# davxy/ark-ec-vrfs

Measured on AMD Instinct MI355X. Metric: Bandersnatch IETF-ECVRF verifies/sec, 2^20 batch per GPU, higher is better.
Workload: dtype u32; 1 GPU; IETF ECVRF verify, Bandersnatch_SHA-512_ELL2, batch 2^20 per GPU, compressed points (161 B/verify), checked decode: on curve + prime-order subgroup, as arkworks' deserialisation, ad="", about 1 in 16 proofs forged (BASELINE.json configs[2]); global_batch=1048576, parallelism=items sharded x1, result gather only, subgroup_check=True

## Files before the change

### ark_ec_vrfs_amd/csrc/fr.cuh

```cuda
#pragma once
#include "fe.cuh"

VRF_NS_BEGIN

template <class C>
VRF_HD void fr_montmul(uint32_t out[8], const uint32_t a[8], const uint32_t b[8]) {
  uint32_t t[10];
#pragma unroll
  for (int i = 0; i < 10; ++i) t[i] = 0;
#pragma unroll
  for (int i = 0; i < 8; ++i) {
    uint64_t c = 0;
#pragma unroll
    for (int j = 0; j < 8; ++j) {
      uint64_t x = (uint64_t)a[j] * b[i] + t[j] + c;
      t[j] = (uint32_t)x;
      c = x >> 32;
    }
    uint64_t x = (uint64_t)t[8] + c;
    t[8] = (uint32_t)x;
    t[9] = (uint32_t)(x >> 32);
    uint32_t m = t[0] * C::R_NINV32;
    c = ((uint64_t)m * C::r32(0) + t[0]) >> 32;
#pragma unroll
// ... 47 lines not shown
  const bool keep = borrow && c == 0;
#pragma unroll
  for (int i = 0; i < 8; ++i) out[i] = keep ? s[i] : d[i];
}

template <class C>
VRF_HD void fr_reduce512(uint32_t out[8], const uint32_t x[16]) {
  uint32_t r1[8], r2[8], lo[8], hi[8];
#pragma unroll
  for (int i = 0; i < 8; ++i) { r1[i] = C::r_r1(i); r2[i] = C::r_r2(i); }
  fr_montmul<C>(lo, x, r1);
  fr_montmul<C>(hi, x + 8, r2);
  fr_add<C>(out, lo, hi);
}

template <class C>
VRF_HD void fr_mul(uint32_t out[8], const uint32_t a[8], const uint32_t b[8]) {
  uint32_t t[8], r2[8];
#pragma unroll
  for (int i = 0; i < 8; ++i) r2[i] = C::r_r2(i);
  fr_montmul<C>(t, a, b);
  fr_montmul<C>(out, t, r2);
}

template <class C>
VRF_HD bool fr_is_canonical(const uint32_t a[8]) {
  bool lt = false, decided = false;
#pragma unroll
  for (int i = 7; i >= 0; --i) {
    uint32_t ri = C::r32(i);
    if (!decided && a[i] != ri) { lt = a[i] < ri; decided = true; }
  }
  return lt;
}

VRF_HD void scalar_recode_signed4(uint32_t out[8], const uint32_t k[8]) {
  uint32_t c = 0;
#pragma unroll
  for (int i = 0; i < 8; ++i) {
    uint64_t x = (uint64_t)k[i] + 0x88888888u + c;
    out[i] = (uint32_t)x;
    c = (uint32_t)(x >> 32);
  }
}
VRF_HD int scalar_digit4(const uint32_t rec[8], int w) {
  uint32_t word = rec[0];
#pragma unroll
  for (int i = 1; i < 8; ++i)
    if ((w >> 3) == i) word = rec[i];
  return (int)((word >> ((w & 7) * 4)) & 15u) - 8;
}

struct GlvHalf {
  uint32_t mag[4];
  bool neg;
};

VRF_HD void acc5_muladd(uint32_t acc[5], const uint32_t x[5], const uint32_t (&y)[5], bool subtract) {
  uint32_t p[5];
  uint64_t carry = 0;
#pragma unroll
  for (int k = 0; k < 5; ++k) {
    uint64_t lo = carry & 0xffffffffu, hi = carry >> 32;
#pragma unroll
    for (int i = 0; i <= k; ++i) {
      uint64_t t = (uint64_t)x[i] * y[k - i];
      lo += t & 0xffffffffu;
      hi += t >> 32;
    }
    p[k] = (uint32_t)lo;
    carry = hi + (lo >> 32);
  }
  uint64_t c = subtract ? 1 : 0;
#pragma unroll
  for (int k = 0; k < 5; ++k) {
    uint64_t t = (uint64_t)acc[k] + (subtract ? ~p[k] : p[k]) + c;
    acc[k] = (uint32_t)t;
    c = t >> 32;
  }
}

VRF_HD void glv_round_mul(uint32_t out[5], const uint32_t k[8], const uint32_t (&g)[5]) {
  uint32_t prod[13];
  uint64_t carry = 0;
#pragma unroll
  for (int col = 0; col < 13; ++col) {
    uint64_t lo = carry & 0xffffffffu, hi = carry >> 32;
#pragma unroll
    for (int i = 0; i < 8; ++i) {
      int j = col - i;
      if (j >= 0 && j < 5) {
        uint64_t t = (uint64_t)k[i] * g[j];
        lo += t & 0xffffffffu;
        hi += t >> 32;
      }
    }
    if (col == 7) lo += 0x80000000u;
    prod[col] = (uint32_t)lo;
    carry = hi + (lo >> 32);
  }
#pragma unroll
  for (int i = 0; i < 5; ++i) out[i] = prod[8 + i];
}

VRF_HD GlvHalf glv_finish(const uint32_t v[5]) {
  GlvHalf h;
  h.neg = (v[4] >> 31) != 0;
  uint64_t c = h.neg ? 1 : 0;
#pragma unroll
  for (int i = 0; i < 4; ++i) {
    uint64_t t = (uint64_t)(h.neg ? ~v[i] : v[i]) + c;
    h.mag[i] = (uint32_t)t;
    c = t >> 32;
  }
  return h;
}

#if VRF_FIELD != 0
VRF_HD void glv_decompose_bs(GlvHalf& k1, GlvHalf& k2, const uint32_t k[8]);
#else
VRF_HD void glv_decompose_bs(GlvHalf& k1, GlvHalf& k2, const uint32_t k[8]) {
  uint32_t c1[5], c2[5];
  glv_round_mul(c1, k, vrfk::BS_GLV_G1);
  glv_round_mul(c2, k, vrfk::BS_GLV_G2);
  uint32_t v1[5], v2[5];
#pragma unroll
  for (int i = 0; i < 5; ++i) { v1[i] = k[i]; v2[i] = 0; }
  acc5_muladd(v1, c1, vrfk::BS_GLV_A1_MAG, !(vrfk::BS_GLV_C1_NEG ^ vrfk::BS_GLV_A1_NEG));
  acc5_muladd(v1, c2, vrfk::BS_GLV_A2_MAG, !(vrfk::BS_GLV_C2_NEG ^ vrfk::BS_GLV_A2_NEG));
  acc5_muladd(v2, c1, vrfk::BS_GLV_B1_MAG, !(vrfk::BS_GLV_C1_NEG ^ vrfk::BS_GLV_B1_NEG));
  acc5_muladd(v2, c2, vrfk::BS_GLV_B2_MAG, !(vrfk::BS_GLV_C2_NEG ^ vrfk::BS_GLV_B2_NEG));
  k1 = glv_finish(v1);
  k2 = glv_finish(v2);
}
#endif

VRF_HD void scalar_recode_signed4_128(uint32_t out[4], const uint32_t k[4]) {
  uint32_t c = 0;
#pragma unroll
  for (int i = 0; i < 4; ++i) {
    uint64_t x = (uint64_t)k[i] + 0x88888888u + c;
    out[i] = (uint32_t)x;
    c = (uint32_t)(x >> 32);
  }
}
VRF_HD int scalar_digit4_128(const uint32_t rec[4], int w) {
  uint32_t word = rec[0];
#pragma unroll
  for (int i = 1; i < 4; ++i)
    if ((w >> 3) == i) word = rec[i];
  return (int)((word >> ((w & 7) * 4)) & 15u) - 8;
}

VRF_NS_END
```

### ark_ec_vrfs_amd/csrc/k_verify.hip

```cpp
#include "kernels.h"
#include "tai_find.cuh"

VRF_NS_BEGIN

template <class S>
VRF_HD void load_cs_reduced(uint32_t c[8], uint32_t s[8]) {
  uint32_t cr[8];
  fr_reduce256<S>(cr, c);
  const bool s_ok = fr_is_canonical<S>(s);
#pragma unroll
  for (int j = 0; j < 8; ++j) { c[j] = s_ok ? cr[j] : 0u; s[j] = s_ok ? s[j] : 0u; }
}

template <class S, int MINW>
__global__ void __launch_bounds__(BLOCK, MINW) k_verify_decode(VerifyArgs a) {
  size_t first = ((size_t)blockIdx.x * BLOCK + threadIdx.x) * a.k_lane;
  if (first >= a.n) return;
  verify_decode_multi<S>(a.k_lane, a.T, first, a.n, a.pk, a.h, a.gamma, a.ws.tabs, a.ws.pts, a.ws.flags, a.check_mask);
}

template <class S>
__global__ void __launch_bounds__(BLOCK, 2) k_verify_input_from_alpha(size_t n, BytesView msg, uint8_t* enc, uint32_t* tabs,
                                                                      DevTables T, const uint8_t* tai_ctr) {
  size_t i = (size_t)blockIdx.x * BLOCK + threadIdx.x;
  if (i >= n) return;
  const uint8_t* m; uint32_t len;
  bytes_get(msg, i, m, len);
  PtE h = data_to_point<S>(m, len, T.sq, tai_ctr ? tai_ctr[i] : 0u);
  FeN x, y;
  te_to_affine(x, y, h);
  uint32_t e[8];
  te_encode_affine(e, x, y, T.sq.str.flags);
  store32(enc, i, e);
  build_glv_tables<S>(tabs + i * (VERIFY_TABS * WIN_TABLE_WORDS) + 2 * WIN_TABLE_WORDS, x, y);
}
template <class S, int MINW>
__global__ void __launch_bounds__(BLOCK, MINW) k_verify_decode_skip_h(VerifyArgs a) {
  size_t first = ((size_t)blockIdx.x * BLOCK + threadIdx.x) * a.k_lane;
  if (first >= a.n) return;
  verify_decode_multi<S, 2, true>(a.k_lane, a.T, first, a.n, a.pk, nullptr, a.gamma, a.ws.tabs, a.ws.pts, a.ws.flags,
                                  a.check_mask);
}

template <class S, int MINW>
__global__ void __launch_bounds__(BLOCK, MINW) k_verify_decode_keyed(VerifyArgs a) {
  size_t first = ((size_t)blockIdx.x * BLOCK + threadIdx.x) * a.k_lane;
  if (first >= a.n) return;
  verify_decode_multi<S, 2>(a.k_lane, a.T, first, a.n, nullptr, a.h, a.gamma, a.ws.tabs, a.ws.pts, a.ws.flags,
                            a.check_mask);
#pragma unroll 1
  for (int k = 0; k < a.k_lane; ++k) {
    const size_t i = first + k;
    if (i >= a.n) break;
    const uint32_t key = a.key_index[i];
    const bool key_ok = key < a.n_keys && a.key_valid[key] != 0;
    if (!key_ok) a.ws.flags[i] = 0;
  }
}

template <class S>
__global__ void __launch_bounds__(BLOCK) k_verify_comb_u(VerifyArgs a) {
  size_t i = (size_t)blockIdx.x * BLOCK + threadIdx.x;
  if (i >= a.n) return;
  uint32_t c[8], s[8];
  load32(c, a.c, i); load32(s, a.s, i);
  load_cs_reduced<S>(c, s);
  const uint32_t key = a.key_index[i] < a.n_keys ? a.key_index[i] : 0;
  PtE r = gcomb_mul<S>(a.T.g_comb, s);
  r = comb_add<S>(r, a.key_combs + (size_t)key * COMB_WORDS, c, true);
  uint32_t* out = a.ws.pts + i * PROVE_PTS_WORDS;
  fe_store(out, r.X); fe_store(out + NL, r.Y); fe_store(out + 2 * NL, r.Z);
}

template <class S>
__global__ void __launch_bounds__(BLOCK) k_verify_decode_affine(VerifyArgs a) {
  size_t i = (size_t)blockIdx.x * BLOCK + threadIdx.x;
  if (i >= a.n) return;
  uint32_t xy[3][16], enc[3][8];
  const uint32_t* p0 = reinterpret_cast<const uint32_t*>(a.pk + i * 64);
  const uint32_t* p1 = reinterpret_cast<const uint32_t*>(a.h + i * 64);
  const uint32_t* p2 = reinterpret_cast<const uint32_t*>(a.gamma + i * 64);
#pragma unroll
  for (int j = 0; j < 16; ++j) { xy[0][j] = p0[j]; xy[1][j] = p1[j]; xy[2][j] = p2[j]; }
  bool ok = verify_decode_affine_item<S>(enc, xy, a.ws.tabs + i * (VERIFY_TABS * WIN_TABLE_WORDS), a.T.sq, a.check_mask,
                                         a.affine_in == 2);
  uint32_t* aux = a.ws.aux + i * AUX_WORDS;
#pragma unroll
  for (int j = 0; j < 8; ++j) { aux[j] = enc[0][j]; aux[8 + j] = enc[1][j]; aux[16 + j] = enc[2][j]; }
  a.ws.flags[i] = ok ? 1 : 0;
}

template <class S, int HALF>
__global__ void __launch_bounds__(BLOCK) k_verify_straus(VerifyArgs a) {
  size_t i = (size_t)blockIdx.x * BLOCK + threadIdx.x;
  if (i >= a.n) return;
  uint32_t c[8], s[8];
  load32(c, a.c, i); load32(s, a.s, i);
  load_cs_reduced<S>(c, s);
  verify_straus_item<S, HALF>(a.ws.pts + i * PROVE_PTS_WORDS + HALF * UV_WORDS, a.T,
                                    a.ws.tabs + i * (VERIFY_TABS * WIN_TABLE_WORDS), c, s);
}

template <class S>
__global__ void __launch_bounds__(BLOCK) k_verify_straus_both(VerifyArgs a) {
  size_t i = (size_t)blockIdx.x * BLOCK + threadIdx.x;
  if (i >= a.n) return;
  uint32_t c[8], s[8];
  load32(c, a.c, i); load32(s, a.s, i);
  load_cs_reduced<S>(c, s);
  const uint32_t* tabs = a.ws.tabs + i * (VERIFY_TABS * WIN_TABLE_WORDS);
  if (blockIdx.y == 0) verify_straus_item<S, 1>(a.ws.pts + i * PROVE_PTS_WORDS + UV_WORDS, a.T, tabs, c, s);
  else verify_straus_item<S, 0>(a.ws.pts + i * PROVE_PTS_WORDS, a.T, tabs, c, s);
}

template <class S, int MINW>
__global__ void __launch_bounds__(BLOCK, MINW) k_verify_finish(VerifyArgs a) {
  size_t first = ((size_t)blockIdx.x * BLOCK + threadIdx.x) * a.k_lane;
  if (first >= a.n) return;
  verify_finish_multi<S>(a.k_lane, first, a.n, a.ws.pts, PROVE_PTS_WORDS, a.pk, a.h, a.gamma,
                         a.affine_in ? a.ws.aux : nullptr, AUX_WORDS, a.c, a.s, a.ad, a.ws.flags, a.status,
                         a.T.sq.str, a.key_index, a.n_keys);
}

template <class S>
static void launch_verify_t(const VerifyArgs& a, hipStream_t st, hipEvent_t* ev) {
  const size_t lanes_k_ = (a.n + a.k_lane - 1) / a.k_lane;
  const dim3 gk = grid_for(lanes_k_);
  if (ev) (void)hipEventRecord(ev[0], st);
  if (a.key_index) VRF_LAUNCH_MINW(k_verify_decode_keyed, S, lanes_k_, gk, spread_lds_bytes(gk.x), st, a);
  else if (a.h_in_tabs) VRF_LAUNCH_MINW(k_verify_decode_skip_h, S, lanes_k_, gk, spread_lds_bytes(gk.x), st, a);
  else if (a.affine_in) hipLaunchKernelGGL(k_verify_decode_affine<S>, grid_for(a.n), dim3(BLOCK), 0, st, a);
  else VRF_LAUNCH_MINW(k_verify_decode, S, lanes_k_, gk, spread_lds_bytes(gk.x), st, a);
  if (!ev && !a.key_index && a.n <= STRAUS_FUSE_MAX_ITEMS) {
    dim3 g2 = grid_for(a.n);
    g2.y = 2;
    hipLaunchKernelGGL(k_verify_straus_both<S>, g2, dim3(BLOCK), 0, st, a);
    if (a.u_out) { launch_test_verify_uv_readout(a, st); return; }
    VRF_LAUNCH_MINW(k_verify_finish, S, lanes_k_, gk, spread_lds_bytes(gk.x), st, a);
    return;
  }
  if (ev) (void)hipEventRecord(ev[1], st);
  hipLaunchKernelGGL((k_verify_straus<S, 1>), grid_for(a.n), dim3(BLOCK), 0, st, a);
  if (ev) (void)hipEventRecord(ev[2], st);
  if (a.key_index) hipLaunchKernelGGL(k_verify_comb_u<S>, grid_for(a.n), dim3(BLOCK), 0, st, a);
  else hipLaunchKernelGGL((k_verify_straus<S, 0>), grid_for(a.n), dim3(BLOCK), 0, st, a);
  if (ev) (void)hipEventRecord(ev[3], st);
  if (a.u_out) { launch_test_verify_uv_readout(a, st); return; }
  VRF_LAUNCH_MINW(k_verify_finish, S, lanes_k_, gk, spread_lds_bytes(gk.x), st, a);
  if (ev) (void)hipEventRecord(ev[4], st);
}
void launch_verify_input_from_alpha(int suite, size_t n, BytesView msg, uint8_t* enc, uint32_t* tabs, DevTables T,
                                    hipStream_t st, uint8_t* tai_ctr, unsigned long long* queue) {
  if (!n) return;
  VRF_DISPATCH_SUITE(suite, {
    const uint8_t* ctr = nullptr;
    if constexpr (!S::H2C_ELL2) {
      if (tai_ctr && queue) { launch_tai_find_t<S>(n, msg, tai_ctr, T.sq, queue, st); ctr = tai_ctr; }
    }
    hipLaunchKernelGGL(k_verify_input_from_alpha<S>, grid_for(n), dim3(BLOCK), 0, st, n, msg, enc, tabs, T, ctr);
  });
}
void launch_ietf_verify(const VerifyArgs& a, hipStream_t st, hipEvent_t* ev) {
  if (a.n == 0) return;
  VRF_DISPATCH_SUITE(a.suite, launch_verify_t<S>(a, st, ev));
}

VRF_NS_END
```

### ark_ec_vrfs_amd/csrc/vrf_core.cuh

```cuda
#pragma once
#include "fe.cuh"
#include "fr.cuh"
#include "sha512.cuh"
#include "te.cuh"

VRF_NS_BEGIN

enum : uint32_t { ST_OK = 0, ST_VERIFICATION_FAILURE = 1, ST_INVALID_DATA = 2 };


constexpr int WIN_ENTRIES = 8;
constexpr int WIN_TABLE_WORDS = WIN_ENTRIES * PTC_WORDS;

enum : int { SUBGROUP_2DESCENT = 0, SUBGROUP_TATE8 = 1, SUBGROUP_ORDER = 2, SUBGROUP_HALVE_TATE4 = 3 };

#if VRF_FIELD == 0
struct SuiteBS : CurveBS {
  static constexpr bool HAS_GLV = true;
  static constexpr int SUBGROUP = SUBGROUP_2DESCENT;
  static constexpr bool H2C_ELL2 = true;
};

struct SuiteJJ : CurveJJ {
  static constexpr bool HAS_GLV = false;
// ... 456 lines not shown
  }
  start = te_add_cached<C>(start, step, false);
  comb_chain<C>(tab + ((size_t)w * GC_COLS + (size_t)seg * GC_SEG) * PTA_WORDS, prefix, start, step, GC_SEG);
}

template <class C>
VRF_HD PtE comb_mul(const uint32_t* comb, const uint32_t k[8]) {
  PtE acc = te_identity();
#pragma unroll 1
  for (int w = 0; w < 32; ++w) {
    uint32_t word = k[0];
#pragma unroll
    for (int i = 1; i < 8; ++i)
      if ((w >> 2) == i) word = k[i];
    uint32_t d = (word >> ((w & 3) * 8)) & 255u;
    uint32_t idx = d ? d - 1 : 0;
    PtA e = pta_load(comb + ((size_t)w * 255 + idx) * PTA_WORDS);
    PtA id = pta_identity();
    bool z = d == 0;
    e.x = fe_select(z, id.x, e.x);
    e.y = fe_select(z, id.y, e.y);
    e.dt = fe_select(z, id.dt, e.dt);
    acc = te_add_affine<C>(acc, e, false);
  }
  return acc;
}

template <class C>
VRF_HD PtE comb_add(PtE acc, const uint32_t* comb, const uint32_t k[8], bool neg = false) {
#pragma unroll 1
  for (int w = 0; w < 32; ++w) {
    uint32_t word = k[0];
#pragma unroll
    for (int i = 1; i < 8; ++i)
      if ((w >> 2) == i) word = k[i];
    uint32_t d = (word >> ((w & 3) * 8)) & 255u;
    uint32_t idx = d ? d - 1 : 0;
    PtA e = pta_load(comb + ((size_t)w * 255 + idx) * PTA_WORDS);
    PtA id = pta_identity();
    bool z = d == 0;
    e.x = fe_select(z, id.x, e.x);
    e.y = fe_select(z, id.y, e.y);
    e.dt = fe_select(z, id.dt, e.dt);
    acc = te_add_affine<C>(acc, e, neg);
  }
  return acc;
}
template <class C>
VRF_HD PtE te_mul_slow(const PtE& base, const uint32_t k[8]) {
  PtE acc = te_identity();
  PtC bc = te_to_cached<C>(base);
#pragma unroll 1
  for (int i = 255; i >= 0; --i) {
    acc = te_dbl<C>(acc, true);
    uint32_t word = k[0];
#pragma unroll
    for (int j = 1; j < 8; ++j)
      if ((i >> 5) == j) word = k[j];
    bool bit = (word >> (i & 31)) & 1u;
    PtE sum = te_add_cached<C>(acc, bc, false);
    acc.X = fe_select(bit, sum.X, acc.X);
    acc.Y = fe_select(bit, sum.Y, acc.Y);
    acc.Z = fe_select(bit, sum.Z, acc.Z);
    acc.T = fe_select(bit, sum.T, acc.T);
  }
  return acc;
}
constexpr int COMB_ROWS = 32, COMB_COLS = 255;
constexpr size_t COMB_WORDS = (size_t)COMB_ROWS * COMB_COLS * PTA_WORDS;
template <class C>
VRF_HD void comb_build_row(uint32_t* row , uint32_t* prefix , const FeN& x, const FeN& y, int w) {
  PtE base = te_from_affine(x, y);
#pragma unroll 1
  for (int i = 0; i < 8 * w; ++i) base = te_dbl<C>(base, i == 8 * w - 1);
  comb_chain<C>(row, prefix, base, te_to_cached<C>(base), COMB_COLS);
}

VRF_HD void enc_canonical(uint32_t w[8]) {
  const uint32_t top = w[7] & 0x7fffffffu;
  uint32_t d1 = (w[0] ^ 1u) | top, dm = (w[0] ^ (vrfk::Q32[0] - 1u)) | (top ^ vrfk::Q32[7]);
#pragma unroll
  for (int i = 1; i < 7; ++i) { d1 |= w[i]; dm |= w[i] ^ vrfk::Q32[i]; }
  if (d1 == 0 || dm == 0) w[7] = top;
}

VRF_HD void u256_shr_bytes(uint32_t w[8], uint32_t nbytes) {
  const uint32_t ws = nbytes >> 2, bs = (nbytes & 3u) * 8u;
  uint32_t t[8];
#pragma unroll
  for (int i = 0; i < 8; ++i) {
    uint32_t lo = 0, hi = 0;
#pragma unroll
    for (int j = 0; j < 8; ++j) {
      if ((uint32_t)j == i + ws) lo = w[j];
      if ((uint32_t)j == i + ws + 1) hi = w[j];
    }
    t[i] = bs ? (lo >> bs) | (hi << (32u - bs)) : lo;
  }
#pragma unroll
  for (int i = 0; i < 8; ++i) w[i] = t[i];
}

template <class S>
VRF_HD void challenge5(uint32_t c_out[8], const uint32_t (&pts)[5][8], const uint8_t* ad,
                       uint32_t ad_len, const SuiteStr& ss) {
  Sha512 h;
  sha512_init(h);
  put_suite_id(h, ss);
  sha512_put_byte(h, 0x02);
  uint64_t w[20];
#pragma unroll
  for (int i = 0; i < 5; ++i) {
    uint32_t e[8];
#pragma unroll
    for (int j = 0; j < 8; ++j) e[j] = pts[i][j];
    enc_canonical(e);
    sha512_words_le32x8(w + 4 * i, e);
  }
  sha512_put_words(h, w);
  sha512_put_bytes(h, ad, ad_len);
  sha512_put_byte(h, 0x00);
  sha512_final(h);
  uint32_t be[8];
  if (ss.flags & SS_CHALLENGE_LE) {
#pragma unroll
    for (int j = 0; j < 8; ++j) {
      const uint32_t w = sha512_word_mem(h, j), have = ss.challenge_len > 4u * j ? ss.challenge_len - 4u * j : 0u;
      be[j] = have >= 4u ? w : have == 0u ? 0u : (w & ((1u << (8u * have)) - 1u));
    }
  } else {
    sha512_be256(be, h);
    if (ss.challenge_len != 32u) u256_shr_bytes(be, 32u - ss.challenge_len);
  }
  fr_reduce256<S>(c_out, be);
}

template <class S>
VRF_HD void proof_challenge_decode(uint32_t out[8], const uint32_t c[8], const SuiteStr& ss) {
  if (ss.challenge_len < 32u) {
#pragma unroll
    for (int j = 0; j < 8; ++j) out[j] = c[j];
  } else {
    fr_reduce256<S>(out, c);
  }
}

constexpr int UV_WORDS = 3 * NL;

VRF_HD FeN fe_sel3(int p, const FeN& a, const FeN& b, const FeN& c) {
  return fe_select(p == 0, a, fe_select(p == 1, b, c));
}

constexpr int VERIFY_TABS = 6;
template <class S>
VRF_HD bool verify_decode_item(const DevTables& T, const uint32_t pk[8], const uint32_t hh[8],
                               const uint32_t gamma[8], uint32_t* tabs, uint32_t check_mask = 0) {
  DecodeA a0 = decode_phase_a<S>(pk), a1 = decode_phase_a<S>(hh), a2 = decode_phase_a<S>(gamma);
  FeN dens[3] = {a0.den, a1.den, a2.den}, dinv[3];
  fe_batch_inv(dinv, dens);
  bool valid = true;
#pragma unroll 1
  for (int p = 0; p < 3; ++p) {
    DecodeA a;
    a.y = fe_sel3(p, a0.y, a1.y, a2.y);
    a.den = fe_sel3(p, a0.den, a1.den, a2.den);
    a.num = fe_select(p == 0, a0.num, fe_select(p == 1, a1.num, a2.num));
    a.flag = p == 0 ? a0.flag : (p == 1 ? a1.flag : a2.flag);
    a.ok = p == 0 ? a0.ok : (p == 1 ? a1.ok : a2.ok);
    FeN di = fe_sel3(p, dinv[0], dinv[1], dinv[2]);
    Fe<1, 4> x;
    valid = decode_phase_b<S>(x, a, di, T.sq) && valid;
    build_glv_tables<S>(tabs + p * 2 * WIN_TABLE_WORDS, x, a.y);
    if ((check_mask >> p) & 1u) valid = in_prime_subgroup<S>(fe_mul(x, fe_one()), a.y, T.sq) && valid;
  }
  return valid;
}

constexpr int VERIFY_K = 8;
constexpr int DEC_SLOT = 4 * NL;

template <class S, int NP = 3, bool SKIP_H = false>
VRF_HD void verify_decode_multi(int K, const DevTables& T, size_t first, size_t n, const uint8_t* pk,
                                const uint8_t* hh, const uint8_t* gamma, uint32_t* tabs_base,
                                uint32_t* scratch_base, uint8_t* flags, uint32_t check_mask = 0) {
  uint32_t* scr = scratch_base + first * (3 * DEC_SLOT);
  FeN run = fe_one();
  uint64_t bits = 0;
#pragma unroll 1
  for (int j = 0; j < NP * K; ++j) {
    const size_t item = first + j / NP;
    const int p = SKIP_H ? (j % NP) * 2 : j % NP + (3 - NP);
    if (item < n) {
      const uint8_t* src = p == 0 ? pk : (p == 1 ? hh : gamma);
      uint32_t enc[8];
      const uint32_t* w = reinterpret_cast<const uint32_t*>(src + item * 32);
#pragma unroll
      for (int k = 0; k < 8; ++k) enc[k] = w[k];
      DecodeA a = decode_phase_a<S>(enc);
      uint32_t* slot = scr + j * DEC_SLOT;
      fe_store(slot, a.y);
      fe_store(slot + NL, a.num);
      fe_store(slot + 2 * NL, a.den);
      fe_store(slot + 3 * NL, run);
      run = fe_mul(run, a.den);
      bits |= (uint64_t)((a.flag ? 1u : 0u) | (a.ok ? 2u : 0u)) << (2 * j);
    }
  }
  FeN inv = fe_inv(run);
  uint32_t valid_mask = 0xffffffffu;
#pragma unroll 1
  for (int j = NP * K - 1; j >= 0; --j) {
    const size_t item = first + j / NP;
    const int p = SKIP_H ? (j % NP) * 2 : j % NP + (3 - NP);
    if (item < n) {
      const uint32_t* slot = scr + j * DEC_SLOT;
      DecodeA a;
      a.y = fe_load<1, 2>(slot);
      a.num = fe_load<1, 6>(slot + NL);
      a.den = fe_load<1, 2>(slot + 2 * NL);
      FeN prefix = fe_load<1, 2>(slot + 3 * NL);
      a.flag = (bits >> (2 * j)) & 1;
      a.ok = (bits >> (2 * j + 1)) & 1;
      FeN di = fe_mul(inv, prefix);
      inv = fe_mul(inv, a.den);
      Fe<1, 4> x;
      bool ok = decode_phase_b<S>(x, a, di, T.sq);
      uint32_t* tab = tabs_base + item * (VERIFY_TABS * WIN_TABLE_WORDS) + p * 2 * WIN_TABLE_WORDS;
      build_glv_tables<S>(tab, x, a.y);
      if ((check_mask >> p) & 1u) ok = in_prime_subgroup<S>(fe_mul(x, fe_one()), a.y, T.sq) && ok;
      if (!ok) valid_mask &= ~(1u << (j / NP));
    }
  }
#pragma unroll 1
  for (int k = 0; k < K; ++k)
    if (first + k < n) flags[first + k] = (valid_mask >> k) & 1;
}

template <class S>
VRF_HD void verify_finish_multi(int K, size_t first, size_t n, uint32_t* pts_base, int pts_stride,
                                const uint8_t* pk, const uint8_t* hh, const uint8_t* gamma,
                                const uint32_t* enc_aux, int aux_stride, const uint8_t* c_arr,
                                const uint8_t* s_arr, const BytesViewLite& ad, const uint8_t* flags,
                                uint8_t* status, const SuiteStr& ss, const uint32_t* key_index = nullptr,
                                size_t n_keys = 0) {
  FeN run = fe_one();
#pragma unroll 1
  for (int j = 0; j < 2 * K; ++j) {
    const size_t item = first + j / 2;
    if (item < n) {
      uint32_t* slot = pts_base + item * pts_stride;
      FeP z = fe_load<1, 5>(slot + (j & 1) * UV_WORDS + 2 * NL);
      fe_store(slot + 2 * UV_WORDS + (j & 1) * NL, run);
      run = fe_mul(run, z);
    }
  }
  FeN inv = fe_inv(run);
  uint32_t encv[8];
#pragma unroll
  for (int k = 0; k < 8; ++k) encv[k] = 0;
#pragma unroll 1
  for (int j = 2 * K - 1; j >= 0; --j) {
    const size_t item = first + j / 2;
    if (item < n) {
      const uint32_t* slot = pts_base + item * pts_stride;
      const uint32_t* uv = slot + (j & 1) * UV_WORDS;
      FeN prefix = fe_load<1, 2>(slot + 2 * UV_WORDS + (j & 1) * NL);
      FeP z = fe_load<1, 5>(uv + 2 * NL);
      FeN zi = fe_mul(inv, prefix);
      inv = fe_mul(inv, z);
      uint32_t e[8];
      te_encode_affine(e, fe_mul(fe_load<1, 5>(uv), zi), fe_mul(fe_load<1, 5>(uv + NL), zi), ss.flags);
      if (j & 1) {
#pragma unroll
        for (int k = 0; k < 8; ++k) encv[k] = e[k];
      } else {
        uint32_t pts[5][8], c[8], sc[8];
        if (enc_aux) {
          const uint32_t* aux = enc_aux + item * aux_stride;
#pragma unroll
          for (int k = 0; k < 8; ++k) { pts[0][k] = aux[k]; pts[1][k] = aux[8 + k]; pts[2][k] = aux[16 + k]; }
        } else {
          size_t pk_row = item;
          if (key_index) pk_row = key_index[item] < n_keys ? key_index[item] : 0;
          const uint32_t* w0 = reinterpret_cast<const uint32_t*>(pk + pk_row * 32);
          const uint32_t* w1 = reinterpret_cast<const uint32_t*>(hh + item * 32);
          const uint32_t* w2 = reinterpret_cast<const uint32_t*>(gamma + item * 32);
#pragma unroll
          for (int k = 0; k < 8; ++k) { pts[0][k] = w0[k]; pts[1][k] = w1[k]; pts[2][k] = w2[k]; }
        }
        const uint32_t* wc = reinterpret_cast<const uint32_t*>(c_arr + item * 32);
        const uint32_t* ws = reinterpret_cast<const uint32_t*>(s_arr + item * 32);
#pragma unroll
        for (int k = 0; k < 8; ++k) { pts[3][k] = e[k]; pts[4][k] = encv[k]; c[k] = wc[k]; sc[k] = ws[k]; }
        const uint8_t* adp; uint32_t adl;
        bytes_lite_get(ad, item, adp, adl);
        uint32_t c2[8], cr[8];
        challenge5<S>(c2, pts, adp, adl, ss);
        proof_challenge_decode<S>(cr, c, ss);
        uint32_t diff = 0;
#pragma unroll
        for (int k = 0; k < 8; ++k) diff |= c2[k] ^ cr[k];
        bool valid = flags[item] != 0 && fr_is_canonical<S>(sc);
        status[item] = (uint8_t)(!valid ? ST_INVALID_DATA : (diff == 0 ? ST_OK : ST_VERIFICATION_FAILURE));
      }
    }
  }
}

template <class S>
VRF_HD bool verify_decode_affine_item(uint32_t enc_out[3][8], const uint32_t (&xy)[3][16], uint32_t* tabs,
                                      const SqrtTables& T, uint32_t check_mask = 0, bool mont256 = false) {
  bool valid = true;
#pragma unroll 1
  for (int p = 0; p < 3; ++p) {
    uint32_t xin[8], yin[8], xw[8], yw[8];
#pragma unroll
    for (int j = 0; j < 8; ++j) {
      xin[j] = p == 0 ? xy[0][j] : p == 1 ? xy[1][j] : xy[2][j];
      yin[j] = p == 0 ? xy[0][8 + j] : p == 1 ? xy[1][8 + j] : xy[2][8 + j];
    }
    valid = valid && !u256_ge(xin, vrfk::Q32) && !u256_ge(yin, vrfk::Q32);
    FeN x = fe_from_abi(xw, xin, mont256), y = fe_from_abi(yw, yin, mont256);
    FeN x2 = fe_sqr(x), y2 = fe_sqr(y), xyv = fe_mul(x, y);
    auto lhs = te_curve_lhs<S>(x2, y2);
    valid = fe_eq(lhs, fe_mul(fe_mul(fe_sqr(xyv), S::d()), fe_one())) && valid;
    build_glv_tables<S>(tabs + p * 2 * WIN_TABLE_WORDS, x, y);
    if ((check_mask >> p) & 1u) valid = in_prime_subgroup<S>(x, y, T) && valid;
    uint32_t e[8];
#pragma unroll
    for (int j = 0; j < 8; ++j) e[j] = yw[j];
    if (te_x_sign(xw, T.str.flags)) e[7] |= 0x80000000u;
#pragma unroll
    for (int j = 0; j < 8; ++j) {
      if (p == 0) enc_out[0][j] = e[j];
      if (p == 1) enc_out[1][j] = e[j];
      if (p == 2) enc_out[2][j] = e[j];
    }
  }
  return valid;
}

template <class S, int HALF>
VRF_HD void verify_straus_item(uint32_t* out_uv, const DevTables& T, const uint32_t* tabs,
                               const uint32_t c[8], const uint32_t s[8]) {
  if constexpr (!S::HAS_GLV) {
    uint32_t recs[8], recc[8];
    scalar_recode_signed4(recs, s);
    scalar_recode_signed4(recc, c);
    PtE r;
    if (HALF == 0) {
      r = win_mul<S, false, true>(tabs, recc, true, challenge_top_window(T.sq.str));
      r = gcomb_add<S, true>(r, T.g_comb, s);
    } else {
      r = straus2<S, true>(tabs + 2 * WIN_TABLE_WORDS, recs, tabs + 4 * WIN_TABLE_WORDS, recc, true, challenge_top_window(T.sq.str));
    }
    fe_store(out_uv, r.X);
    fe_store(out_uv + NL, r.Y);
    fe_store(out_uv + 2 * NL, r.Z);
    return;
  } else {
  Straus4 q;
  GlvHalf h[4];
  glv_decompose_bs(h[0], h[1], c);
#pragma unroll
  for (int t = 0; t < 2; ++t) {
    scalar_recode_signed4_128(q.rec[t], h[t].mag);
    q.neg[t] = !h[t].neg;
  }
  PtE r;
  if (HALF == 0) {
    q.tab[0] = tabs; q.tab[1] = tabs + WIN_TABLE_WORDS;
    q.tab[2] = tabs; q.tab[3] = tabs;
#pragma unroll
    for (int i = 0; i < 4; ++i) { q.rec[2][i] = 0; q.rec[3][i] = 0; }
    q.neg[2] = false; q.neg[3] = false;
    r = straus4<S, 2, false, true>(q);
    r = gcomb_add<S, true>(r, T.g_comb, s);
  } else {
    glv_decompose_bs(h[2], h[3], s);
#pragma unroll
    for (int t = 2; t < 4; ++t) {
      scalar_recode_signed4_128(q.rec[t], h[t].mag);
      q.neg[t] = h[t].neg;
    }
    q.tab[0] = tabs + 4 * WIN_TABLE_WORDS; q.tab[1] = tabs + 5 * WIN_TABLE_WORDS;
    q.tab[2] = tabs + 2 * WIN_TABLE_WORDS; q.tab[3] = tabs + 3 * WIN_TABLE_WORDS;
    r = straus4<S, 4, false, true>(q);
  }
  fe_store(out_uv, r.X);
  fe_store(out_uv + NL, r.Y);
  fe_store(out_uv + 2 * NL, r.Z);
  }
}

template <class S>
VRF_HD uint32_t verify_finish_item(const uint32_t* uv, const uint32_t pk[8], const uint32_t hh[8],
                                   const uint32_t gamma[8], const uint32_t c[8],
                                   const uint32_t s[8], bool valid, const uint8_t* ad,
                                   uint32_t ad_len, const SuiteStr& ss) {
  valid = valid && fr_is_canonical<S>(s);
  uint32_t cr[8];
  proof_challenge_decode<S>(cr, c, ss);
  FeP zin[2] = {fe_load<1, 5>(uv + 2 * NL), fe_load<1, 5>(uv + UV_WORDS + 2 * NL)};
  FeN zi[2];
  fe_batch_inv(zi, zin);
  uint32_t pts[5][8];
#pragma unroll
  for (int i = 0; i < 8; ++i) { pts[0][i] = pk[i]; pts[1][i] = hh[i]; pts[2][i] = gamma[i]; }
  te_encode_affine(pts[3], fe_mul(fe_load<1, 5>(uv), zi[0]), fe_mul(fe_load<1, 5>(uv + NL), zi[0]), ss.flags);
  te_encode_affine(pts[4], fe_mul(fe_load<1, 5>(uv + UV_WORDS), zi[1]),
                   fe_mul(fe_load<1, 5>(uv + UV_WORDS + NL), zi[1]), ss.flags);
  uint32_t c2[8];
  challenge5<S>(c2, pts, ad, ad_len, ss);
  uint32_t diff = 0;
#pragma unroll
  for (int i = 0; i < 8; ++i) diff |= c2[i] ^ cr[i];
  if (!valid) return ST_INVALID_DATA;
  return diff == 0 ? ST_OK : ST_VERIFICATION_FAILURE;
}

VRF_HD void put_dst_prime(Sha512& h, const SuiteStr& ss) { sha512_put_packed(h, ss.dst_prime_w, ss.dst_prime_len); }

template <class S>
VRF_HD void expand_message_xmd96(uint64_t (&hb)[2][8], const uint8_t* msg, uint32_t msg_len, const SuiteStr& ss) {
  Sha512 b0;
  sha512_init(b0);
#pragma unroll
  for (int i = 0; i < 6; ++i) sha512_put(b0, 0, 8);
  sha512_put_bytes(b0, msg, msg_len);
  sha512_put_byte(b0, 0x00);
  sha512_put_byte(b0, 0x60);
  sha512_put_byte(b0, 0x00);
  put_dst_prime(b0, ss);
  sha512_final(b0);
  uint64_t h0[8], h1[8];
#pragma unroll
  for (int i = 0; i < 8; ++i) h0[i] = b0.h[i];
#pragma unroll
  for (int i = 0; i < 8; ++i) h1[i] = 0;
#pragma unroll 1
  for (int t = 0; t < 2; ++t) {
    Sha512 b;
    sha512_init(b);
#pragma unroll
    for (int i = 0; i < 8; ++i) sha512_put(b, h0[i] ^ h1[i], 8);
    sha512_put_byte(b, (uint8_t)(t + 1));
    put_dst_prime(b, ss);
    sha512_final(b);
#pragma unroll
    for (int i = 0; i < 8; ++i) {
      if (t == 0) { h1[i] = b.h[i]; hb[0][i] = b.h[i]; } else { hb[1][i] = b.h[i]; }
    }
  }
}

template <class S>
VRF_HD void hash_to_field2(Fe<1, 4>& u0, Fe<1, 4>& u1, const uint8_t* msg, uint32_t msg_len, const SuiteStr& ss) {
  uint64_t hb[2][8];
  expand_message_xmd96<S>(hb, msg, msg_len, ss);
  uint32_t w0[16], w1[16];
#pragma unroll
  for (int i = 0; i < 16; ++i) { w0[i] = 0; w1[i] = 0; }
#pragma unroll
  for (int j = 0; j < 6; ++j) {
    uint64_t a = hb[0][j];
    uint64_t b = (j < 2) ? hb[0][6 + j] : hb[1][j - 2];
    w0[2 * (5 - j)] = (uint32_t)a; w0[2 * (5 - j) + 1] = (uint32_t)(a >> 32);
    w1[2 * (5 - j)] = (uint32_t)b; w1[2 * (5 - j) + 1] = (uint32_t)(b >> 32);
  }
  u0 = fe_from_u512(w0);
  u1 = fe_from_u512(w1);
}

VRF_HD bool fe_parity(const FeN& a) {
  uint32_t w[8];
  fe_to_u256(w, a);
  return w[0] & 1;
}

#if VRF_FIELD == 0
template <class S>
VRF_HD PtE ell2_map(const Fe<1, 4>& u, const FeN& Dinv, const SqrtTables& T) {
  const FeN JK = fe_const(vrfk::BS_ELL2_JK_M), K2I = fe_const(vrfk::BS_ELL2_K2I_M);
  const FeN K = fe_const(vrfk::BS_ELL2_K_M);
  FeN x1 = fe_mul(fe_const(vrfk::BS_ELL2_NJK_M), Dinv);
  FeN t = fe_mul(fe_add(x1, JK), x1);
  FeN gx1 = fe_mul(fe_add(t, K2I), x1);
  FeN root;
  bool sq = fe_sqrt_or_zsqrt(root, gx1, T);
  uint32_t rw[8];
  fe_to_u256(rw, root);
  uint32_t nz = 0;
#pragma unroll
  for (int i = 0; i < 8; ++i) nz |= rw[i];
  sq = sq || (nz == 0);
  Fe<1, 8> x2 = fe_norm(fe_neg(fe_norm(fe_add(x1, JK))));
  FeN y2 = fe_mul(root, u);
  Fe<1, 8> x1w = x1;
  Fe<1, 8> x = fe_select(sq, x1w, x2);
  FeN y = fe_select(sq, root, y2);
  bool odd = fe_parity(y);
  auto ys = fe_norm(fe_cneg(odd != sq, y));
  FeN s = fe_mul(x, K), tt = fe_mul(ys, K);
  auto sp1 = fe_add(s, fe_one());
  auto sm1 = fe_sub(s, fe_one());
  PtE p;
  p.X = fe_mul(s, sp1);
  p.Y = fe_mul(sm1, tt);
  p.Z = fe_mul(tt, sp1);
  p.T = fe_mul(s, sm1);
  bool exc = fe_is_zero(p.Z);
  PtE id = te_identity();
  p.X = fe_select(exc, id.X, p.X);
  p.Y = fe_select(exc, id.Y, p.Y);
  p.Z = fe_select(exc, id.Z, p.Z);
  p.T = fe_select(exc, id.T, p.T);
  return p;
}

template <class S>
VRF_HD PtE hash_to_curve_ell2(const uint8_t* msg, uint32_t msg_len, const SqrtTables& T) {
  Fe<1, 4> u[2];
  hash_to_field2<S>(u[0], u[1], msg, msg_len, T.str);
  FeN D[2], Di[2];
#pragma unroll
  for (int i = 0; i < 2; ++i) {
    FeN d = fe_canon(fe_add(fe_mul5(fe_sqr(u[i])), fe_one()));
    bool dz = true;
#pragma unroll
    for (int k = 0; k < NL; ++k) dz = dz && (d.v[k] == 0);
    D[i] = fe_select(dz, fe_one(), d);
  }
  fe_batch_inv(Di, D);
  PtE q0 = te_identity();
  PtE acc = te_identity();
#pragma unroll 1
  for (int i = 0; i < 2; ++i) {
    Fe<1, 4> ui = fe_select(i == 0, u[0], u[1]);
    FeN di = fe_select(i == 0, Di[0], Di[1]);
    PtE q = ell2_map<S>(ui, di, T);
    if (i == 0) q0 = q; else acc = te_add<S>(q0, q);
  }
#pragma unroll 1
  for (int i = 0; i < S::COFACTOR_LOG2; ++i) acc = te_dbl<S>(acc, true);
  return acc;
// ... 643 lines not shown
```

Baseline: 28.02 million verifies/s.

## Replace GLV Straus windows with joint-table ladders for verify multi-scalar muls

For GLV suites, verification now builds joint precomputed tables instead of per-point window tables. The U half uses a 12-entry joint table of Y and psi(Y) with signed 2-bit digits. The V half uses a 15-entry table of all subset sums of ±H, ±psi(H), ±Gamma, ±psi(Gamma) and runs a single-bit joint ladder over 127 bits with one add per bit. Table construction now needs c and s at decode time, so the scalars are loaded and GLV-decomposed inside the decode kernels. The aim is fewer point additions and smaller tables per item, at the cost of more doublings and extra decode-stage work.

```diff
diff --git a/ark_ec_vrfs_amd/csrc/fr.cuh b/ark_ec_vrfs_amd/csrc/fr.cuh
--- a/ark_ec_vrfs_amd/csrc/fr.cuh
+++ b/ark_ec_vrfs_amd/csrc/fr.cuh
@@ -223,4 +223,31 @@
   return (int)((word >> ((w & 7) * 4)) & 15u) - 8;
 }
 
+constexpr uint32_t GLV_HALF_TOP_WORD_CAP = 0x77777777u;
+static_assert(GLV_HALF_TOP_WORD_CAP < 0x80000000u, "bit 127 of a GLV half must be clear: the joint ladders start at bit 126");
+
+VRF_HD int scalar_bit_128(const uint32_t k[4], int bit) {
+  uint32_t word = k[0];
+#pragma unroll
+  for (int i = 1; i < 4; ++i)
+    if ((bit >> 5) == i) word = k[i];
+  return (int)((word >> (bit & 31)) & 1u);
+}
+VRF_HD void scalar_recode_signed2_128(uint32_t out[4], const uint32_t k[4]) {
+  uint32_t c = 0;
+#pragma unroll
+  for (int i = 0; i < 4; ++i) {
+    uint64_t x = (uint64_t)k[i] + 0x55555555u + c;
+    out[i] = (uint32_t)x;
+    c = (uint32_t)(x >> 32);
+  }
+}
+VRF_HD int scalar_digit2_128(const uint32_t rec[4], int w) {
+  uint32_t word = rec[0];
+#pragma unroll
+  for (int i = 1; i < 4; ++i)
+    if ((w >> 4) == i) word = rec[i];
+  return (int)((word >> ((w & 15) * 2)) & 3u) - 1;
+}
+
 VRF_NS_END
diff --git a/ark_ec_vrfs_amd/csrc/k_verify.hip b/ark_ec_vrfs_amd/csrc/k_verify.hip
--- a/ark_ec_vrfs_amd/csrc/k_verify.hip
+++ b/ark_ec_vrfs_amd/csrc/k_verify.hip
@@ -3,20 +3,13 @@
 
 VRF_NS_BEGIN
 
-template <class S>
-VRF_HD void load_cs_reduced(uint32_t c[8], uint32_t s[8]) {
-  uint32_t cr[8];
-  fr_reduce256<S>(cr, c);
-  const bool s_ok = fr_is_canonical<S>(s);
-#pragma unroll
-  for (int j = 0; j < 8; ++j) { c[j] = s_ok ? cr[j] : 0u; s[j] = s_ok ? s[j] : 0u; }
-}
 
 template <class S, int MINW>
 __global__ void __launch_bounds__(BLOCK, MINW) k_verify_decode(VerifyArgs a) {
   size_t first = ((size_t)blockIdx.x * BLOCK + threadIdx.x) * a.k_lane;
   if (first >= a.n) return;
-  verify_decode_multi<S>(a.k_lane, a.T, first, a.n, a.pk, a.h, a.gamma, a.ws.tabs, a.ws.pts, a.ws.flags, a.check_mask);
+  verify_decode_multi<S, 3, false, S::HAS_GLV>(a.k_lane, a.T, first, a.n, a.pk, a.h, a.gamma, a.ws.tabs, a.ws.pts, a.ws.flags,
+                                               a.check_mask, a.c, a.s);
 }
 
 template <class S>
@@ -32,22 +25,23 @@
   uint32_t e[8];
   te_encode_affine(e, x, y, T.sq.str.flags);
   store32(enc, i, e);
-  build_glv_tables<S>(tabs + i * (VERIFY_TABS * WIN_TABLE_WORDS) + 2 * WIN_TABLE_WORDS, x, y);
+  if constexpr (S::HAS_GLV) jt_park_xy(tabs + i * (VERIFY_TABS * WIN_TABLE_WORDS) + JT_HXY, x, y);
+  else build_glv_tables<S>(tabs + i * (VERIFY_TABS * WIN_TABLE_WORDS) + 2 * WIN_TABLE_WORDS, x, y);
 }
 template <class S, int MINW>
 __global__ void __launch_bounds__(BLOCK, MINW) k_verify_decode_skip_h(VerifyArgs a) {
   size_t first = ((size_t)blockIdx.x * BLOCK + threadIdx.x) * a.k_lane;
   if (first >= a.n) return;
-  verify_decode_multi<S, 2, true>(a.k_lane, a.T, first, a.n, a.pk, nullptr, a.gamma, a.ws.tabs, a.ws.pts, a.ws.flags,
-                                  a.check_mask);
+  verify_decode_multi<S, 2, true, S::HAS_GLV>(a.k_lane, a.T, first, a.n, a.pk, nullptr, a.gamma, a.ws.tabs, a.ws.pts,
+                                              a.ws.flags, a.check_mask, a.c, a.s);
 }
 
 template <class S, int MINW>
 __global__ void __launch_bounds__(BLOCK, MINW) k_verify_decode_keyed(VerifyArgs a) {
   size_t first = ((size_t)blockIdx.x * BLOCK + threadIdx.x) * a.k_lane;
   if (first >= a.n) return;
-  verify_decode_multi<S, 2>(a.k_lane, a.T, first, a.n, nullptr, a.h, a.gamma, a.ws.tabs, a.ws.pts, a.ws.flags,
-                            a.check_mask);
+  verify_decode_multi<S, 2, false, S::HAS_GLV>(a.k_lane, a.T, first, a.n, nullptr, a.h, a.gamma, a.ws.tabs, a.ws.pts,
+                                               a.ws.flags, a.check_mask, a.c, a.s);
 #pragma unroll 1
   for (int k = 0; k < a.k_lane; ++k) {
     const size_t i = first + k;
@@ -82,8 +76,13 @@
   const uint32_t* p2 = reinterpret_cast<const uint32_t*>(a.gamma + i * 64);
 #pragma unroll
   for (int j = 0; j < 16; ++j) { xy[0][j] = p0[j]; xy[1][j] = p1[j]; xy[2][j] = p2[j]; }
-  bool ok = verify_decode_affine_item<S>(enc, xy, a.ws.tabs + i * (VERIFY_TABS * WIN_TABLE_WORDS), a.T.sq, a.check_mask,
-                                         a.affine_in == 2);
+  uint32_t c[8], s[8];
+  if constexpr (S::HAS_GLV) {
+    load32(c, a.c, i); load32(s, a.s, i);
+    load_cs_reduced<S>(c, s);
+  }
+  bool ok = verify_decode_affine_item<S, S::HAS_GLV>(enc, xy, a.ws.tabs + i * (VERIFY_TABS * WIN_TABLE_WORDS), a.T.sq,
+                                                     a.check_mask, a.affine_in == 2, c, s);
   uint32_t* aux = a.ws.aux + i * AUX_WORDS;
 #pragma unroll
   for (int j = 0; j < 8; ++j) { aux[j] = enc[0][j]; aux[8 + j] = enc[1][j]; aux[16 + j] = enc[2][j]; }
@@ -97,8 +96,10 @@
   uint32_t c[8], s[8];
   load32(c, a.c, i); load32(s, a.s, i);
   load_cs_reduced<S>(c, s);
-  verify_straus_item<S, HALF>(a.ws.pts + i * PROVE_PTS_WORDS + HALF * UV_WORDS, a.T,
-                                    a.ws.tabs + i * (VERIFY_TABS * WIN_TABLE_WORDS), c, s);
+  uint32_t* out = a.ws.pts + i * PROVE_PTS_WORDS + HALF * UV_WORDS;
+  const uint32_t* tabs = a.ws.tabs + i * (VERIFY_TABS * WIN_TABLE_WORDS);
+  if constexpr (S::HAS_GLV) verify_joint_item<S, HALF>(out, a.T, tabs, c, s);
+  else verify_straus_item<S, HALF>(out, a.T, tabs, c, s);
 }
 
 template <class S>
@@ -109,8 +110,13 @@
   load32(c, a.c, i); load32(s, a.s, i);
   load_cs_reduced<S>(c, s);
   const uint32_t* tabs = a.ws.tabs + i * (VERIFY_TABS * WIN_TABLE_WORDS);
-  if (blockIdx.y == 0) verify_straus_item<S, 1>(a.ws.pts + i * PROVE_PTS_WORDS + UV_WORDS, a.T, tabs, c, s);
-  else verify_straus_item<S, 0>(a.ws.pts + i * PROVE_PTS_WORDS, a.T, tabs, c, s);
+  if constexpr (S::HAS_GLV) {
+    if (blockIdx.y == 0) verify_joint_item<S, 1>(a.ws.pts + i * PROVE_PTS_WORDS + UV_WORDS, a.T, tabs, c, s);
+    else verify_joint_item<S, 0>(a.ws.pts + i * PROVE_PTS_WORDS, a.T, tabs, c, s);
+  } else {
+    if (blockIdx.y == 0) verify_straus_item<S, 1>(a.ws.pts + i * PROVE_PTS_WORDS + UV_WORDS, a.T, tabs, c, s);
+    else verify_straus_item<S, 0>(a.ws.pts + i * PROVE_PTS_WORDS, a.T, tabs, c, s);
+  }
 }
 
 template <class S, int MINW>
diff --git a/ark_ec_vrfs_amd/csrc/vrf_core.cuh b/ark_ec_vrfs_amd/csrc/vrf_core.cuh
--- a/ark_ec_vrfs_amd/csrc/vrf_core.cuh
+++ b/ark_ec_vrfs_amd/csrc/vrf_core.cuh
@@ -632,6 +632,127 @@
 }
 
 constexpr int VERIFY_TABS = 6;
+
+template <class S>
+VRF_HD void load_cs_reduced(uint32_t c[8], uint32_t s[8]) {
+  uint32_t cr[8];
+  fr_reduce256<S>(cr, c);
+  const bool s_ok = fr_is_canonical<S>(s);
+#pragma unroll
+  for (int j = 0; j < 8; ++j) { c[j] = s_ok ? cr[j] : 0u; s[j] = s_ok ? s[j] : 0u; }
+}
+
+constexpr int JT_Y_ENTRIES = 12, JT_V_ENTRIES = 15;
+constexpr int JT_Y = 0;
+constexpr int JT_V = JT_Y + JT_Y_ENTRIES * PTC_WORDS;
+constexpr int JT_EXT = JT_V + JT_V_ENTRIES * PTC_WORDS;
+constexpr int JT_YEXT = JT_EXT + 8 * PTC_WORDS;
+constexpr int JT_HXY = JT_YEXT + 2 * PTC_WORDS;
+constexpr int JT_GXY = JT_HXY + 2 * NL;
+static_assert(JT_GXY + 2 * NL <= VERIFY_TABS * WIN_TABLE_WORDS, "the joint tables and their parking fit the item's region");
+
+VRF_HD void pte_store(uint32_t* m, const PtE& p) {
+  fe_store(m, p.X); fe_store(m + NL, p.Y); fe_store(m + 2 * NL, p.Z); fe_store(m + 3 * NL, p.T);
+}
+VRF_HD PtE pte_load(const uint32_t* m) {
+  PtE p;
+  p.X = fe_load<1, 5>(m); p.Y = fe_load<1, 5>(m + NL); p.Z = fe_load<1, 5>(m + 2 * NL); p.T = fe_load<1, 5>(m + 3 * NL);
+  return p;
+}
+VRF_HD void jt_park_xy(uint32_t* m, const Fe<1, 4>& x, const FeN& y) { fe_store(m, x); fe_store(m + NL, y); }
+
+#if VRF_FIELD == 0
+template <class C>
+VRF_HD PtE te_psi_signed(const PtE& p, bool neg) {
+  const FeN b = fe_const(vrfk::BS_PSI_B_M);
+  const auto c = fe_norm(fe_cneg(neg, fe_const(vrfk::BS_PSI_C_M)));
+  auto YY = fe_sqr(p.Y);
+  auto ZZ = fe_sqr(p.Z);
+  auto XY = fe_mul(p.X, p.Y);
+  auto bZZ = fe_mul(ZZ, b);
+  auto A = fe_sub(ZZ, YY);
+  auto Bv = fe_sub(YY, bZZ);
+  auto Cv = fe_add(YY, bZZ);
+  auto cA = fe_mul(A, c);
+  auto bC = fe_mul(Cv, b);
+  PtE r;
+  r.X = fe_mul(cA, Bv);
+  r.Y = fe_mul(bC, XY);
+  r.Z = fe_mul(XY, Bv);
+  r.T = fe_mul(cA, bC);
+  bool exc = fe_is_zero(r.Z);
+  PtE id = te_identity();
+  r.X = fe_select(exc, id.X, r.X);
+  r.Y = fe_select(exc, id.Y, r.Y);
+  r.Z = fe_select(exc, id.Z, r.Z);
+  r.T = fe_select(exc, id.T, r.T);
+  return r;
+}
+#else
+template <class C>
+VRF_HD PtE te_psi_signed(const PtE& p, bool neg);
+#endif
+
+template <class S>
+VRF_HD void build_joint_y_table(uint32_t* reg, const FeP& x, const FeP& y) {
+  const PtE p = te_from_affine(x, y);
+  const PtE q = te_psi<S>(p);
+#pragma unroll 1
+  for (int t = 0; t < 2; ++t) {
+    PtE b;
+    b.X = fe_select(t == 0, p.X, q.X); b.Y = fe_select(t == 0, p.Y, q.Y);
+    b.Z = fe_select(t == 0, p.Z, q.Z); b.T = fe_select(t == 0, p.T, q.T);
+    const PtE d = te_dbl<S>(b, true);
+    ptc_store(reg + JT_Y + 2 * t * PTC_WORDS, te_to_cached<S>(b));
+    ptc_store(reg + JT_Y + (2 * t + 1) * PTC_WORDS, te_to_cached<S>(d));
+    if (t == 0) { pte_store(reg + JT_YEXT, b); pte_store(reg + JT_YEXT + PTC_WORDS, d); }
+  }
+#pragma unroll 1
+  for (int i = 0; i < 8; ++i) {
+    const PtE e = pte_load(reg + JT_YEXT + (i >> 2) * PTC_WORDS);
+    const PtC c = ptc_load(reg + JT_Y + (2 + ((i >> 1) & 1)) * PTC_WORDS);
+    ptc_store(reg + JT_Y + (4 + i) * PTC_WORDS, te_to_cached<S>(te_add_cached<S>(e, c, (i & 1) != 0)));
+  }
+}
+VRF_HD int joint_y_index(int a, int b, bool& neg) {
+  neg = a < 0 || (a == 0 && b < 0);
+  if (neg) { a = -a; b = -b; }
+  const int bm = b < 0 ? -b : b;
+  if (a == 0) return bm == 0 ? 0 : 2 + bm;
+  if (bm == 0) return a;
+  return 5 + ((a - 1) << 2) + ((bm - 1) << 1) + (b < 0 ? 1 : 0);
+}
+
+template <class S>
+VRF_HD void build_joint_v_table(uint32_t* reg, const uint32_t c[8], const uint32_t s[8]) {
+  GlvHalf h[4];
+  glv_decompose_bs(h[0], h[1], c);
+  glv_decompose_bs(h[2], h[3], s);
+  const bool neg0 = !h[0].neg, neg1 = !h[1].neg, neg2 = h[2].neg, neg3 = h[3].neg;
+#pragma unroll 1
+  for (int p = 0; p < 2; ++p) {
+    const uint32_t* xy = reg + (p == 0 ? JT_GXY : JT_HXY);
+    const bool nb = p == 0 ? neg0 : neg2, npsi = p == 0 ? neg1 : neg3;
+    const FeN x = fe_mul(fe_cneg(nb, fe_load<1, 4>(xy)), fe_one());
+    const PtE b = te_from_affine(x, fe_load<1, 2>(xy + NL));
+    const PtE q = te_psi_signed<S>(b, nb != npsi);
+    const int m = 1 << (2 * p);
+    ptc_store(reg + JT_V + (m - 1) * PTC_WORDS, te_to_cached<S>(b));
+    ptc_store(reg + JT_V + (2 * m - 1) * PTC_WORDS, te_to_cached<S>(q));
+    pte_store(reg + JT_EXT + (m - 1) * PTC_WORDS, b);
+    pte_store(reg + JT_EXT + (2 * m - 1) * PTC_WORDS, q);
+  }
+#pragma unroll 1
+  for (int m = 3; m < 16; ++m) {
+    if ((m & (m - 1)) == 0) continue;
+    const int top = m >= 8 ? 8 : (m >= 4 ? 4 : 2);
+    const PtE e = te_add_cached<S>(pte_load(reg + JT_EXT + (m - top - 1) * PTC_WORDS),
+                                   ptc_load(reg + JT_V + (top - 1) * PTC_WORDS), false);
+    ptc_store(reg + JT_V + (m - 1) * PTC_WORDS, te_to_cached<S>(e));
+    if (m < 8) pte_store(reg + JT_EXT + (m - 1) * PTC_WORDS, e);
+  }
+}
+
 template <class S>
 VRF_HD bool verify_decode_item(const DevTables& T, const uint32_t pk[8], const uint32_t hh[8],
                                const uint32_t gamma[8], uint32_t* tabs, uint32_t check_mask = 0) {
@@ -659,10 +780,11 @@
 constexpr int VERIFY_K = 8;
 constexpr int DEC_SLOT = 4 * NL;
 
-template <class S, int NP = 3, bool SKIP_H = false>
+template <class S, int NP = 3, bool SKIP_H = false, bool JOINT = false>
 VRF_HD void verify_decode_multi(int K, const DevTables& T, size_t first, size_t n, const uint8_t* pk,
                                 const uint8_t* hh, const uint8_t* gamma, uint32_t* tabs_base,
-                                uint32_t* scratch_base, uint8_t* flags, uint32_t check_mask = 0) {
+                                uint32_t* scratch_base, uint8_t* flags, uint32_t check_mask = 0,
+                                const uint8_t* c_arr = nullptr, const uint8_t* s_arr = nullptr) {
   uint32_t* scr = scratch_base + first * (3 * DEC_SLOT);
   FeN run = fe_one();
   uint64_t bits = 0;
@@ -705,8 +827,23 @@
       inv = fe_mul(inv, a.den);
       Fe<1, 4> x;
       bool ok = decode_phase_b<S>(x, a, di, T.sq);
-      uint32_t* tab = tabs_base + item * (VERIFY_TABS * WIN_TABLE_WORDS) + p * 2 * WIN_TABLE_WORDS;
-      build_glv_tables<S>(tab, x, a.y);
+      if constexpr (JOINT) {
+        uint32_t* reg = tabs_base + item * (VERIFY_TABS * WIN_TABLE_WORDS);
+        if (p == 0) build_joint_y_table<S>(reg, x, a.y);
+        else jt_park_xy(reg + (p == 1 ? JT_HXY : JT_GXY), x, a.y);
+        if (p == (SKIP_H ? 2 : 1)) {
+          uint32_t c[8], s[8];
+          const uint32_t* wc = reinterpret_cast<const uint32_t*>(c_arr + item * 32);
+          const uint32_t* ws = reinterpret_cast<const uint32_t*>(s_arr + item * 32);
+#pragma unroll
+          for (int k = 0; k < 8; ++k) { c[k] = wc[k]; s[k] = ws[k]; }
+          load_cs_reduced<S>(c, s);
+          build_joint_v_table<S>(reg, c, s);
+        }
+      } else {
+        uint32_t* tab = tabs_base + item * (VERIFY_TABS * WIN_TABLE_WORDS) + p * 2 * WIN_TABLE_WORDS;
+        build_glv_tables<S>(tab, x, a.y);
+      }
       if ((check_mask >> p) & 1u) ok = in_prime_subgroup<S>(fe_mul(x, fe_one()), a.y, T.sq) && ok;
       if (!ok) valid_mask &= ~(1u << (j / NP));
     }
@@ -787,9 +924,10 @@
   }
 }
 
-template <class S>
+template <class S, bool JOINT = false>
 VRF_HD bool verify_decode_affine_item(uint32_t enc_out[3][8], const uint32_t (&xy)[3][16], uint32_t* tabs,
-                                      const SqrtTables& T, uint32_t check_mask = 0, bool mont256 = false) {
+                                      const SqrtTables& T, uint32_t check_mask = 0, bool mont256 = false,
+                                      const uint32_t* c = nullptr, const uint32_t* s = nullptr) {
   bool valid = true;
 #pragma unroll 1
   for (int p = 0; p < 3; ++p) {
@@ -804,7 +942,12 @@
     FeN x2 = fe_sqr(x), y2 = fe_sqr(y), xyv = fe_mul(x, y);
     auto lhs = te_curve_lhs<S>(x2, y2);
     valid = fe_eq(lhs, fe_mul(fe_mul(fe_sqr(xyv), S::d()), fe_one())) && valid;
-    build_glv_tables<S>(tabs + p * 2 * WIN_TABLE_WORDS, x, y);
+    if constexpr (JOINT) {
+      if (p == 0) build_joint_y_table<S>(tabs, x, y);
+      else jt_park_xy(tabs + (p == 1 ? JT_HXY : JT_GXY), x, y);
+    } else {
+      build_glv_tables<S>(tabs + p * 2 * WIN_TABLE_WORDS, x, y);
+    }
     if ((check_mask >> p) & 1u) valid = in_prime_subgroup<S>(x, y, T) && valid;
     uint32_t e[8];
 #pragma unroll
@@ -817,6 +960,7 @@
       if (p == 2) enc_out[2][j] = e[j];
     }
   }
+  if constexpr (JOINT) build_joint_v_table<S>(tabs, c, s);
   return valid;
 }
 
@@ -871,6 +1015,65 @@
   fe_store(out_uv + NL, r.Y);
   fe_store(out_uv + 2 * NL, r.Z);
   }
+}
+
+template <class S>
+VRF_HD PtE joint_u_ladder(const uint32_t* ytab, const GlvHalf& c1, const GlvHalf& c2) {
+  uint32_t r1[4], r2[4];
+  scalar_recode_signed2_128(r1, c1.mag);
+  scalar_recode_signed2_128(r2, c2.mag);
+  const bool n1 = !c1.neg, n2 = !c2.neg;
+  PtE acc = te_identity();
+#pragma unroll 1
+  for (int w = 63; w >= 0; --w) {
+    if (w != 63) {
+#pragma unroll 1
+      for (int j = 0; j < 2; ++j) acc = te_dbl<S, true>(acc, j == 1);
+    }
+    const int d1 = scalar_digit2_128(r1, w), d2 = scalar_digit2_128(r2, w);
+    bool neg;
+    const int idx = joint_y_index(n1 ? -d1 : d1, n2 ? -d2 : d2, neg);
+    acc = te_add_cached<S, true>(acc, win_lookup(ytab, idx), neg, w == 0);
+  }
+  return acc;
+}
+VRF_HD int joint_v_index(const uint32_t (&m)[4][4], int bit) {
+  return scalar_bit_128(m[0], bit) | (scalar_bit_128(m[1], bit) << 1) | (scalar_bit_128(m[2], bit) << 2) |
+         (scalar_bit_128(m[3], bit) << 3);
+}
+template <class S>
+VRF_HD PtE joint_v_ladder(const uint32_t* vtab, const uint32_t (&m)[4][4]) {
+  const PtC first = win_lookup(vtab, joint_v_index(m, 126));
+  PtE acc;
+  acc.X = first.X; acc.Y = first.Y; acc.Z = first.Z; acc.T = fe_zero();
+#pragma unroll 1
+  for (int bit = 125; bit >= 0; --bit) {
+    acc = te_dbl<S, true>(acc, true);
+    acc = te_add_cached<S, true>(acc, win_lookup(vtab, joint_v_index(m, bit)), false, false);
+  }
+  return acc;
+}
+template <class S, int HALF>
+VRF_HD void verify_joint_item(uint32_t* out_uv, const DevTables& T, const uint32_t* reg, const uint32_t c[8],
+                              const uint32_t s[8]) {
+  GlvHalf h[4];
+  glv_decompose_bs(h[0], h[1], c);
+  PtE r;
+  if (HALF == 0) {
+    r = joint_u_ladder<S>(reg + JT_Y, h[0], h[1]);
+    r = gcomb_add<S, true>(r, T.g_comb, s);
+  } else {
+    glv_decompose_bs(h[2], h[3], s);
+    uint32_t m[4][4];
+#pragma unroll
+    for (int t = 0; t < 4; ++t)
+#pragma unroll
+      for (int i = 0; i < 4; ++i) m[t][i] = h[t].mag[i];
+    r = joint_v_ladder<S>(reg + JT_V, m);
+  }
+  fe_store(out_uv, r.X);
+  fe_store(out_uv + NL, r.Y);
+  fe_store(out_uv + 2 * NL, r.Z);
 }
 
 template <class S>
```

After: 29.13 million verifies/s (median of 6 runs). +3.9%, better.
